# acbull/pyHGT

Hardware: AMD Instinct MI355X
Metric: HGTConv forward edges/sec (higher is better)
Workload: dtype f32 (typed linears and relation transforms as 3-term fp16 hi/lo MFMA with power-of-two row scales, fp32 accumulate)

## Files before the change

include/hgt_hip.h:

```cpp
#ifndef HGT_HIP_H_
#define HGT_HIP_H_

#include <stddef.h>
#include <stdint.h>

#ifdef __cplusplus
extern "C" {
#endif

#define HGT_ABI_VERSION 8

#define HGT_OK 0
#define HGT_ERR_INVALID_ARG (-1)
#define HGT_ERR_UNSUPPORTED (-2)
#define HGT_ERR_WORKSPACE (-3)
#define HGT_ERR_TOO_LARGE (-4)
#define HGT_ERR_LAUNCH (-5)

#define HGT_RTE_LEN 240

const char* hgt_strerror(int code);
int hgt_abi_version(void);
#define HGT_FEATURE_DETERMINISTIC_TRAINING 2
int hgt_build_features(void);
// ... 76 lines not shown
int hgt_linear_update_f16x3(const float* agg, int64_t ld_agg, const int32_t* rows, const int32_t* group_off,
                            int32_t n_groups, int64_t n_rows, int32_t k, int32_t n_out, const void* w_split,
                            const float* bias, int64_t b_group_stride, const float* x_skip, int64_t ld_skip,
                            const float* skip, const float* ln_w, const float* ln_b, int32_t use_norm, float* out,
                            void* stream);
int hgt_zero_rows(const int32_t* rows, const int32_t* range, int32_t d, float* out, void* stream);

int hgt_relation_pack(const float* relation_att, const float* relation_msg, const float* relation_pri,
                      int32_t n_relations, int32_t n_heads, int32_t n_heads_layout, int32_t d_k, int32_t dk_pad,
                      float* att_t, float* msg_p, void* stream);

int hgt_edge_logits(const void* plan, int64_t n_nodes, int64_t n_edges, int32_t n_types, int32_t n_relations,
                    int32_t n_heads, int32_t dk_pad, const float* Q, const float* K, const float* rte_k,
                    const float* att_t, float* logits, void* stream);
int hgt_edge_logits_mfma(const void* plan, int64_t n_nodes, int64_t n_edges, int32_t n_types, int32_t n_relations,
                         int32_t n_heads, int32_t dk_pad, const float* Q, const float* K, const float* rte_k,
                         const float* att_t, const void* att_frag, int32_t frag_f16, float* logits, void* stream);
int hgt_relation_kside_bytes(int32_t n_relations, int32_t n_heads, int32_t dk_pad, uint64_t* out_host);
int hgt_relation_kside_pack(const float* att_t, int32_t n_relations, int32_t n_heads, int32_t dk_pad, void* att_kside, void* stream);
int hgt_edge_logits_kside(const void* plan, int64_t n_nodes, int64_t n_edges, int32_t n_types, int32_t n_relations,
                          int32_t n_heads, int32_t dk_pad, const float* Q, const float* K, const float* rte_k,
                          const float* att_t, const void* att_kside, int32_t frag_f16, float* logits, void* stream);
int hgt_kside_image_map(int32_t n_blocks, int32_t* image_map, int32_t* b_col, int32_t* c_out);
int hgt_edge_logits_range(const void* plan, int64_t n_nodes, int64_t n_edges, int32_t n_types, int32_t n_relations,
                          int32_t n_heads, int32_t dk_pad, const float* Q, const float* K, const float* rte_k,
                          const float* att_t, const void* att_frag, int32_t frag_f16, float* logits, int32_t item_begin,
                          int32_t item_end, void* stream);
int hgt_edge_softmax(const void* plan, int64_t n_nodes, int64_t n_edges, int32_t n_types, int32_t n_relations,
                     int32_t n_heads, float* logits_att, void* stream);
int hgt_edge_aggregate(const void* plan, int64_t n_nodes, int64_t n_edges, int32_t n_types, int32_t n_relations,
                       int32_t n_heads, int32_t dk_pad, const float* logits, const float* V, const float* rte_v,
                       const float* msg_p, const void* msg_frag, float* agg, int64_t n_q_rows, int32_t apply_gelu,
                       void* hub_ws, void* stream);
int hgt_edge_aggregate_items_bytes(int64_t n_edges, int32_t n_heads, int32_t dk_pad, uint64_t* out_host);
int hgt_edge_aggregate_items(const void* plan, int64_t n_nodes, int64_t n_edges, int32_t n_types, int32_t n_relations,
                             int32_t n_heads, int32_t dk_pad, const float* logits, const float* V, const float* rte_v,
                             const void* msg_frag, int32_t frag_f16, float* agg, int64_t n_q_rows, int32_t apply_gelu,
                             void* scratch, uint64_t scratch_bytes, void* stream);
int hgt_edge_aggregate_items_update(const void* plan, int64_t n_nodes, int64_t n_edges, int32_t n_types, int32_t n_relations,
                                    int32_t n_heads, int32_t dk_pad, const float* logits, const float* V, const float* rte_v,
                                    const void* msg_frag, int32_t frag_f16, int64_t n_q_rows, void* scratch, uint64_t scratch_bytes,
                                    const int32_t* rows, const int32_t* group_off, int32_t n_groups, const void* w_a_split,
                                    const float* b_a, const float* x_skip, int64_t ld_skip, const float* skip, const float* ln_w,
                                    const float* ln_b, int32_t use_norm, int32_t n_out, float* out, void* stream);
int hgt_edge_logits_slice(const void* plan, int64_t n_nodes, int64_t n_edges, int32_t n_types, int32_t n_relations,
                          int32_t n_heads, int32_t dk_pad, const float* Q, const float* K, const float* rte_k,
// ... 169 lines not shown
    int32_t stage;
    const int32_t* proj_rows;
    const int32_t* proj_off;
    int64_t proj_n;
    void* prepared;
    uint64_t prepared_bytes;
    int32_t prepared_valid;
    int32_t plan_no_hubs;
    int32_t flags;
    int32_t slice_index;
    int32_t slice_count;
    int64_t q_begin, q_end;
    int32_t item_begin, item_end;
    const void* proj_c24;
    int64_t proj_c24_row0;
} hgt_conv_args;

#define HGT_FLAG_NO_FUSED_UPDATE 1
#define HGT_FLAG_VALU_AGGREGATE  2
#define HGT_FLAG_MFMA_LOGITS     4
#define HGT_FLAG_VALU_LOGITS     8
#define HGT_FLAG_KSIDE_LOGITS 65536
#define HGT_FLAG_NO_KSIDE_LOGITS 131072
#define HGT_FLAG_ITEM_AGGREGATE 16
#define HGT_FLAG_NO_ITEM_AGGREGATE 32
#define HGT_FLAG_FUSED_ANY_SIZE 64
#define HGT_FLAG_XS_GEMM_ALWAYS 1024
#define HGT_FLAG_XS_GEMM_NEVER 2048
#define HGT_FLAG_NO_TILE_GEMM 4096
#define HGT_FLAG_NO_MERGE_UPDATE 8192
#define HGT_FLAG_NO_COOP_EDGE 16384
#define HGT_FLAG_COOP_EDGE_ALWAYS 32768
#define HGT_FLAG_DETERMINISTIC_HUBS 128

#define HGT_N_PHASE_EVENTS 7

int hgt_conv_workspace_bytes(int64_t n_nodes, int64_t n_edges, int32_t in_dim, int32_t out_dim,
                             int32_t n_types, int32_t n_relations, int32_t n_heads, int32_t use_rte,
                             uint64_t* out_host);
int hgt_conv_workspace_bytes_ex(int64_t n_nodes, int64_t n_edges, int32_t in_dim, int32_t out_dim,
                                int32_t n_types, int32_t n_relations, int32_t n_heads, int32_t use_rte, int32_t options,
                                uint64_t* out_host);
int hgt_conv_prepared_bytes(int32_t in_dim, int32_t out_dim, int32_t n_types, int32_t n_relations, int32_t n_heads,
                            int32_t use_rte, uint64_t* out_host);
int hgt_conv_forward(const hgt_conv_args* args_host, void* stream);

// ... 181 lines not shown
```

pyhgt_amd/_lib.py:

```python
import ctypes as C
import os

_HERE = os.path.dirname(os.path.abspath(__file__))
LIB_PATH = os.environ.get("HGT_LIB_PATH", os.path.join(_HERE, "lib", "libhgt_hip.so"))

HGT_RTE_LEN = 240
HGT_N_PHASE_EVENTS = 7
HGT_FLAG_NO_FUSED_UPDATE = 1
HGT_FLAG_VALU_AGGREGATE = 2
HGT_FLAG_MFMA_LOGITS = 4
HGT_FLAG_VALU_LOGITS = 8
HGT_FLAG_ITEM_AGGREGATE = 16
HGT_FLAG_NO_ITEM_AGGREGATE = 32
HGT_FLAG_FUSED_ANY_SIZE = 64
HGT_FLAG_DETERMINISTIC_HUBS = 128
HGT_FLAG_XS_GEMM_ALWAYS = 1024
HGT_FLAG_XS_GEMM_NEVER = 2048
HGT_FLAG_NO_TILE_GEMM = 4096
HGT_FLAG_NO_MERGE_UPDATE = 8192
HGT_FLAG_NO_COOP_EDGE = 16384
HGT_FLAG_COOP_EDGE_ALWAYS = 32768
HGT_FLAG_KSIDE_LOGITS = 65536
HGT_FLAG_NO_KSIDE_LOGITS = 131072
HGT_LINEAR_FORCE_XS = 0x100
HGT_LINEAR_NO_XS = 0x200
HGT_LINEAR_NO_TILE = 0x400
HGT_LINEAR_TANH = 0x1000
HGT_FEATURE_DETERMINISTIC_TRAINING = 2
HGT_STACK_MAX_PIECES = 256
HGT_SAMPLER_MAX_TYPES = 16
HGT_SAMPLER_MAX_TRIPLES = 48
HGT_SAMPLER_MAX_NUMBER = 1024
HGT_SAMPLER_HUB_DEG = 512
HGT_SAMPLER_TIME_NONE = -2 ** 31
HGT_SAMPLER_MAX_BATCH = 64


class HgtLayout(C.Structure):
    _fields_ = [("d_k", C.c_int32), ("dk_pad", C.c_int32), ("d_pad", C.c_int32), ("vec", C.c_int32), ("heads", C.c_int32)]


class HgtPlanSizes(C.Structure):
    _fields_ = [("plan_bytes", C.c_uint64), ("tmp_bytes", C.c_uint64), ("max_items", C.c_int64), ("n_bins", C.c_int64)]


class HgtPlanRows(C.Structure):
# ... 73 lines not shown
    "hgt_plan_from_sorted": (C.c_int, [_vp, _vp, _vp, _vp, _vp, _i64, _i64, _i64, _i32, _i32, _vp, _u64, _vp, _u64, _vp]),
    "hgt_typed_linear": (C.c_int, [_vp, _i64, _vp, _vp, _i32, _i64, _i32, _i32, _vp, _i64, _vp, _i64, _vp, _vp, _vp,
                                   _i32, _i32, _i32, _i32, _vp]),
    "hgt_split_weights_bytes": (C.c_int, [_i32, _i32, _i32, C.POINTER(_u64)]),
    "hgt_split_weights": (C.c_int, [_vp, _i64, _i32, _i32, _i32, _vp, _vp]),
    "hgt_typed_linear_bf16x3": (C.c_int, [_vp, _i64, _vp, _vp, _i32, _i64, _i32, _i32, _vp, _vp, _i64, _vp, _vp, _vp,
                                          _i32, _i32, _i32, _vp]),
    "hgt_linear_update_bf16x3": (C.c_int, [_vp, _i64, _vp, _vp, _i32, _i64, _i32, _i32, _vp, _vp, _i64, _vp, _i64, _vp, _vp, _vp,
                                           _i32, _vp, _vp]),
    "hgt_split_weights_f16": (C.c_int, [_vp, _i64, _i32, _i32, _i32, _vp, _vp]),
    "hgt_typed_linear_xs_schedule": (C.c_int, [_vp, _i32, _i64, _i32, _i32, _vp, _i64, C.POINTER(_i64)]),
    "hgt_typed_linear_f16x3": (C.c_int, [_vp, _i64, _vp, _vp, _i32, _i64, _i32, _i32, _vp, _vp, _i64, _vp, _vp, _vp,
                                         _i32, _i32, _i32, _vp]),
    "hgt_linear_update_f16x3": (C.c_int, [_vp, _i64, _vp, _vp, _i32, _i64, _i32, _i32, _vp, _vp, _i64, _vp, _i64, _vp, _vp, _vp,
                                          _i32, _vp, _vp]),
    "hgt_zero_rows": (C.c_int, [_vp, _vp, _i32, _vp, _vp]),
    "hgt_relation_pack": (C.c_int, [_vp, _vp, _vp, _i32, _i32, _i32, _i32, _i32, _vp, _vp, _vp]),
    "hgt_edge_logits": (C.c_int, [_vp, _i64, _i64, _i32, _i32, _i32, _i32, _vp, _vp, _vp, _vp, _vp, _vp]),
    "hgt_edge_logits_mfma": (C.c_int, [_vp, _i64, _i64, _i32, _i32, _i32, _i32, _vp, _vp, _vp, _vp, _vp, _i32, _vp, _vp]),
    "hgt_relation_kside_bytes": (C.c_int, [_i32, _i32, _i32, C.POINTER(_u64)]),
    "hgt_relation_kside_pack": (C.c_int, [_vp, _i32, _i32, _i32, _vp, _vp]),
    "hgt_edge_logits_kside": (C.c_int, [_vp, _i64, _i64, _i32, _i32, _i32, _i32, _vp, _vp, _vp, _vp, _vp, _i32, _vp, _vp]),
    "hgt_kside_image_map": (C.c_int, [_i32, _vp, _vp, _vp]),
    "hgt_edge_logits_range": (C.c_int, [_vp, _i64, _i64, _i32, _i32, _i32, _i32, _vp, _vp, _vp, _vp, _vp, _i32, _vp, _i32, _i32, _vp]),
    "hgt_edge_aggregate_update_range": (C.c_int, [_vp, _i64, _i64, _i32, _i32, _i32, _i32, _vp, _vp, _vp, _vp, _vp, _vp, _i64, _vp, _vp, _vp,
                                                  _vp, _vp, _vp, _i64, _vp, _vp, _vp, _i32, _i32, _vp, _vp, _i64, _i64, _i32, _i32]),
    "hgt_hub_workspace_bytes_ex": (C.c_int, [_i64, _i32, _i32, _i32, _i32, C.POINTER(_u64)]),
    "hgt_edge_aggregate_ex": (C.c_int, [_vp, _i64, _i64, _i32, _i32, _i32, _i32, _vp, _vp, _vp, _vp, _vp, _i32, _vp, _i64, _i32, _vp, _i32, _vp]),
    "hgt_edge_logits_slice": (C.c_int, [_vp, _i64, _i64, _i32, _i32, _i32, _i32, _vp, _vp, _vp, _vp, _vp, _i32, _i32, _vp]),
    "hgt_edge_aggregate_slice": (C.c_int, [_vp, _i64, _i64, _i32, _i32, _i32, _i32, _vp, _vp, _vp, _vp, _vp, _vp, _i64, _i32, _vp,
                                           _i32, _i32, _vp, _i32, _i32, _vp]),
    "hgt_edge_aggregate_slice_ex": (C.c_int, [_vp, _i64, _i64, _i32, _i32, _i32, _i32, _vp, _vp, _vp, _vp, _vp, _vp, _i64, _i32, _vp,
                                              _i32, _i32, _vp, _i32, _i32, _i32, _vp]),
    "hgt_edge_softmax": (C.c_int, [_vp, _i64, _i64, _i32, _i32, _i32, _vp, _vp]),
    "hgt_edge_aggregate": (C.c_int, [_vp, _i64, _i64, _i32, _i32, _i32, _i32, _vp, _vp, _vp, _vp, _vp, _vp, _i64, _i32, _vp, _vp]),
    "hgt_edge_aggregate_f16x3": (C.c_int, [_vp, _i64, _i64, _i32, _i32, _i32, _i32, _vp, _vp, _vp, _vp, _vp, _vp, _i64, _i32, _vp, _vp]),
    "hgt_relation_frag_pack_f16": (C.c_int, [_vp, _i32, _i32, _i32, _vp, _vp]),
    "hgt_edge_aggregate_items_bytes": (C.c_int, [_i64, _i32, _i32, C.POINTER(_u64)]),
    "hgt_edge_spmm_items": (C.c_int, [_vp, _i64, _i64, _i32, _i32, _i32, _i32, _vp, _vp, _vp, _vp, _vp, _i64, _i64, _vp, _u64, _vp]),
    "hgt_edge_aggregate_items_update": (C.c_int, [_vp, _i64, _i64, _i32, _i32, _i32, _i32, _vp, _vp, _vp, _vp, _i32, _i64, _vp, _u64, _vp, _vp, _i32,
                                                  _vp, _vp, _vp, _i64, _vp, _vp, _vp, _i32, _i32, _vp, _vp]),
    "hgt_edge_aggregate_items": (C.c_int, [_vp, _i64, _i64, _i32, _i32, _i32, _i32, _vp, _vp, _vp, _vp, _i32, _vp, _i64, _i32, _vp, _u64, _vp]),
    "hgt_plan_header_to_host": (C.c_int, [_vp, _vp, _vp]),
    "hgt_relation_frag_bytes": (C.c_int, [_i32, _i32, _i32, C.POINTER(_u64)]),
    "hgt_relation_frag_pack": (C.c_int, [_vp, _i32, _i32, _i32, _vp, _vp]),
    "hgt_hub_workspace_bytes": (C.c_int, [_i64, _i32, _i32, C.POINTER(_u64)]),
# ... 127 lines not shown
```

pyhgt_amd/csrc/hgt_api.hip:

```cpp
#include "hgt_common.h"

#ifndef HGT_FUSED_MIN_NODES
#define HGT_FUSED_MIN_NODES 16384
#endif
#ifndef HGT_ITEM_AGG_MAX_NODES
#define HGT_ITEM_AGG_MAX_NODES 65536
#endif
#ifndef HGT_ITEM_AGG_DEFAULT_NODES
#define HGT_ITEM_AGG_DEFAULT_NODES 65536
#endif

int hgt_edge_logits_kside_items(const void* plan, int64_t N, int64_t E, int32_t T, int32_t R, int32_t H, int32_t dk_pad, const float* Q,
                                const float* K, const float* rte_k, const void* att_kside, float* logits, int item_lo, int item_hi, void* stream);

namespace {

struct ConvWorkspace {
    uint64_t off_q, off_k, off_v, off_logits, off_agg, off_trans, off_att_t, off_msg_p, off_msg_f, off_att_f, off_att_k, off_hub;
    uint64_t off_rte_lin, off_rte_k, off_rte_v, off_rte_rows, off_rte_off, off_ws_qkv, off_ws_a, off_ws_rte, off_off2, off_pending, off_state, off_zitems, zitems_bytes, total;
    void drop_item_scratch() { zitems_bytes = 0; total = off_zitems; }
};

static ConvWorkspace conv_workspace(int64_t N, int64_t NQ, int64_t E, int in_dim, int out_dim, int T, int R, int , int use_rte,
                                    const hgt_layout& lay, bool item_scratch = true, bool det_hubs = false) {
    const int H = lay.heads;
    ConvWorkspace w;
    uint64_t o = 0;
    auto take = [&](uint64_t bytes) { uint64_t r = o; o = hgt_align_up(o + bytes, 256); return r; };
    const uint64_t dp = (uint64_t)lay.d_pad;
    w.off_q = take((uint64_t)NQ * dp * 4);
    w.off_k = take((uint64_t)N * dp * 4);
    w.off_v = take((uint64_t)N * dp * 4);
    w.off_logits = take((uint64_t)E * H * 4);
    w.off_agg = take((uint64_t)NQ * dp * 4);
    w.off_trans = take((uint64_t)NQ * out_dim * 4);
    w.off_att_t = take((uint64_t)R * H * lay.dk_pad * lay.dk_pad * 4);
// ... 273 lines not shown
                          a->b_qkv, 3 * dp, Q, K, V, dp, 0, ws_qkv, 0, !fresh);
        int rc = linear(a->x, din, pr.rows_q, pr.off_q, T, NQ, din, dp, a->w_qkv, wstride, a->b_qkv, 3 * dp, Q, nullptr, nullptr, dp, 0, ws_a);
        if (rc != HGT_OK) return rc;
        rc = linear(a->x, din, pr.rows_all, pr.off_all, T, N, din, 2 * dp, a->w_qkv + (int64_t)dp * din, wstride, a->b_qkv + dp, 3 * dp,
                    K, V, nullptr, dp, 0, wb + w.off_ws_qkv);
        if (rc != HGT_OK || !(a->prepared && fresh && split)) return rc;
        return split_weights(a->w_qkv, wstride, T, din, 3 * dp, ws_qkv, stream);
    }

    int temporal_tables() const {
        if (!a->use_rte || !fresh) return HGT_OK;
        float* rte_lin = (float*)(wb + w.off_rte_lin);
        int32_t* rrows = (int32_t*)(wb + w.off_rte_rows);
        int32_t* roff = (int32_t*)(wb + w.off_rte_off);
        k_rte_row_lists<<<(T * HGT_RTE_LEN + 255) / 256, 256, 0, stream>>>(T, rrows, roff);
        int rc = linear(a->rte_emb, din, rrows, roff, 1, HGT_RTE_LEN, din, din, a->rte_w, 0, a->rte_b, 0, rte_lin, nullptr, nullptr, din, 1,
                        wb + w.off_ws_rte);
        if (rc != HGT_OK) return rc;
        return linear(rte_lin, din, rrows, roff, T, (int64_t)T * HGT_RTE_LEN, din, 2 * dp, a->w_qkv + (int64_t)dp * din, (int64_t)3 * dp * din,
                      nullptr, 0, rte_k, rte_v, nullptr, dp, 1, ws_a);
    }

    int edge_logits() const {
        if (r.logits == LOGITS_KSIDE) {
            const int rc = hgt_edge_logits_kside(a->plan, N, E, T, R, H, dkp, Q, K, rte_k, att_t, att_k_buf, fmode, logits, stream);
            if (rc != HGT_ERR_UNSUPPORTED) return rc;
            if (r.mfma_logits) return hgt_edge_logits_mfma(a->plan, N, E, T, R, H, dkp, Q, K, rte_k, att_t, att_f_buf, fmode, logits, stream);
        }
        switch (r.logits) {
            case LOGITS_RANGE:
                if (r.kside_range) {
                    const int rc = hgt_edge_logits_kside_items(a->plan, N, E, T, R, H, dkp, Q, K, rte_k, att_k_buf, logits, a->item_begin, a->item_end, stream);
                    if (rc != HGT_ERR_UNSUPPORTED) return rc;
                }
                return hgt_edge_logits_range(a->plan, N, E, T, R, H, dkp, Q, K, rte_k, att_t, r.mfma_logits ? att_f_buf : nullptr, fmode, logits,
                                             a->item_begin, a->item_end, stream);
            case LOGITS_SLICE: return hgt_edge_logits_slice(a->plan, N, E, T, R, H, dkp, Q, K, rte_k, att_t, logits, sl_lo, sl_hi, stream);
            case LOGITS_MFMA: return hgt_edge_logits_mfma(a->plan, N, E, T, R, H, dkp, Q, K, rte_k, att_t, att_f_buf, fmode, logits, stream);
            default: return hgt_edge_logits(a->plan, N, E, T, R, H, dkp, Q, K, rte_k, att_t, logits, stream);
        }
    }

    int aggregate_update(int64_t q0, int64_t q1, int hub_det) const {
        return hgt_edge_aggregate_update_sel(a->plan, N, E, T, R, H, dkp, logits, V, rte_v, msg_p, msg_f, agg, NQ, hub_ws,
                                             (int32_t*)(wb + w.off_pending), a->node_type, ws_upd, a->b_a, a->x, din, a->skip, a->ln_w,
                                             a->ln_b, a->use_norm, dout, a->out, stream, q0, q1, f16 ? 1 : 0, hub_det);
    }

    int aggregate(AggForm form) const {
        void* zitems = wb + w.off_zitems;
        switch (form) {
            case AGG_FUSED:
                if (det_hubs && hub_ws && !msg_f)
                    return HGT_ERR_UNSUPPORTED;
                return aggregate_update(0, (det_hubs && hub_ws) ? NQ : -1, (det_hubs && hub_ws) ? 1 : 0);
// ... 164 lines not shown
```

pyhgt_amd/csrc/hgt_edge_logits_kside.hip:

```cpp
#include "hgt_edge_common.h"
#include "hgt_split_common.h"
#include "hgt_kside_map.h"

namespace {

typedef unsigned hgt_u32x2 __attribute__((ext_vector_type(2)));

__device__ __forceinline__ void half_pair(unsigned x, unsigned& lo, unsigned& up) {
#if __has_builtin(__builtin_amdgcn_permlane32_swap)
    const hgt_u32x2 r = __builtin_amdgcn_permlane32_swap(x, x, false, false);
    lo = r[0];
    up = r[1];
#else
    const unsigned o = (unsigned)__shfl_xor((int)x, 32);
    const bool upper = (threadIdx.x & 32) != 0;
    lo = upper ? o : x;
    up = upper ? x : o;
#endif
}
__device__ __forceinline__ unsigned half_max_bits(unsigned x) {
    unsigned a, b;
    half_pair(x, a, b);
    return max(a, b);
}
// ... 30 lines not shown
    const float* blk = attT + (int64_t)rh * HGT_KSIDE_DK * HGT_KSIDE_DK;
    unsigned m = 0u;
#pragma unroll
    for (int q = 0; q < 4; ++q) m = max(m, __builtin_bit_cast(unsigned, fabsf(blk[t + 256 * q])));
    m = wave_max_bits(m);
    if ((t & 63) == 0) s_m[t >> 6] = m;
    __syncthreads();
    m = max(max(s_m[0], s_m[1]), max(s_m[2], s_m[3]));
    const int e = kside_exp(m);
    const float scale = kside_scale(e);
#pragma unroll
    for (int q = 0; q < 4; ++q) {
        const int p = t + 256 * q;
        const int j = p & 7, lane = (p >> 3) & 63, s = p >> 9;
        const float v = blk[hgt_kside_image_out(lane) * HGT_KSIDE_DK + hgt_kside_image_k(s, lane, j)];
        unsigned short hi, lo;
        split1_t<true>(v, scale, hi, lo);
        img[hgt_kside_image_index(rh, s, 0, lane, j)] = hi;
        img[hgt_kside_image_index(rh, s, 1, lane, j)] = lo;
    }
    if (t == 0) reinterpret_cast<int*>(img + (int64_t)n_rh * HGT_KSIDE_BLOCK_ELEMS)[rh] = e - 141;
}

struct KsideRows {
    float4 k[4], q[4];
};

typedef unsigned hgt_u32x4 __attribute__((ext_vector_type(4)));
typedef __amdgpu_buffer_rsrc_t kside_rsrc;

__device__ __forceinline__ kside_rsrc kside_table(const float* p, unsigned bytes) {
    return __builtin_amdgcn_make_buffer_rsrc(const_cast<float*>(p), 0, (int)bytes, 0x00020000);
}
__device__ __forceinline__ float4 kside_load16(kside_rsrc t, unsigned off) {
    const hgt_u32x4 v = __builtin_amdgcn_raw_buffer_load_b128(t, (int)off, 0, 0);
    return __builtin_bit_cast(float4, v);
}

template <int H>
__device__ __forceinline__ void kside_issue(kside_rsrc K, kside_rsrc Q, unsigned koff, unsigned qoff, int h, KsideRows& b) {
#pragma unroll
    for (int i = 0; i < 4; ++i) b.k[i] = kside_load16(K, koff + h * 128 + 16 * i);
#pragma unroll
    for (int i = 0; i < 4; ++i) b.q[i] = kside_load16(Q, qoff + h * 128 + 16 * i);
}

__device__ __forceinline__ float kside_head(const KsideRows& b, const hgt_f16x8 (&ah)[2], const hgt_f16x8 (&al)[2], int ea) {
    const int ek = kside_exp(half_max_bits(abs_bits16(b.k)));
    const float ks = kside_scale(ek);
    hgt_f16x8 kh[2], kl[2];
#pragma unroll
    for (int s = 0; s < 2; ++s) {
        static_assert(hgt_kside_k_col(1, 0, 0) == 8 && hgt_kside_k_col(0, 1, 0) == 16, "k-step s takes floats 8 s .. 8 s + 7 of the lane's piece");
        uint4 hi, lo;
        split2_f16(b.k[2 * s].x * ks, b.k[2 * s].y * ks, hi.x, lo.x);
        split2_f16(b.k[2 * s].z * ks, b.k[2 * s].w * ks, hi.y, lo.y);
        split2_f16(b.k[2 * s + 1].x * ks, b.k[2 * s + 1].y * ks, hi.z, lo.z);
        split2_f16(b.k[2 * s + 1].z * ks, b.k[2 * s + 1].w * ks, hi.w, lo.w);
        kh[s] = __builtin_bit_cast(hgt_f16x8, hi);
        kl[s] = __builtin_bit_cast(hgt_f16x8, lo);
    }
    f32x16 acc = {0.f, 0.f, 0.f, 0.f, 0.f, 0.f, 0.f, 0.f, 0.f, 0.f, 0.f, 0.f, 0.f, 0.f, 0.f, 0.f};
    acc = __builtin_amdgcn_mfma_f32_32x32x16_f16(al[0], kh[0], acc, 0, 0, 0);
    acc = __builtin_amdgcn_mfma_f32_32x32x16_f16(al[1], kh[1], acc, 0, 0, 0);
    acc = __builtin_amdgcn_mfma_f32_32x32x16_f16(ah[0], kl[0], acc, 0, 0, 0);
    acc = __builtin_amdgcn_mfma_f32_32x32x16_f16(ah[1], kl[1], acc, 0, 0, 0);
    acc = __builtin_amdgcn_mfma_f32_32x32x16_f16(ah[0], kh[0], acc, 0, 0, 0);
    acc = __builtin_amdgcn_mfma_f32_32x32x16_f16(ah[1], kh[1], acc, 0, 0, 0);
    int eq = (int)(half_max_bits(abs_bits16(b.q)) >> 23);
    eq = eq < 1 ? 1 : (eq > 253 ? 253 : eq);
    const float qs = __builtin_bit_cast(float, (unsigned)(254 - eq) << 23);
    static_assert(hgt_kside_c_out(1, 5) == 21, "register reg of the accumulator is output 16 half + reg: the lane's own Q piece");
    const hgt_f32x2 qs2 = {qs, qs};
    hgt_f32x2 d = {0.0f, 0.0f};
#pragma unroll
    for (int i = 0; i < 4; ++i) {
        const hgt_f32x2 q0 = {b.q[i].x, b.q[i].y}, q1 = {b.q[i].z, b.q[i].w};
        const hgt_f32x2 a0 = {acc[4 * i], acc[4 * i + 1]}, a1 = {acc[4 * i + 2], acc[4 * i + 3]};
        d = __builtin_elementwise_fma(q0 * qs2, a0, d);
        d = __builtin_elementwise_fma(q1 * qs2, a1, d);
    }
    const float d0 = d[0], d1 = d[1];
    return ldexpf(half_sum(d0 + d1), (eq - 127) + (ek - 141) + ea);
}

template <int H>
__global__ __launch_bounds__(256, 2) void k_edge_logits_kside(
    const HgtItem* __restrict__ items, const HgtPlanHeader* __restrict__ hdr, const int32_t* __restrict__ esrc,
    const int32_t* __restrict__ edst, const float* __restrict__ Qp, const float* __restrict__ Kp, unsigned table_bytes,
    const unsigned short* __restrict__ img, float* __restrict__ logits, int R, int item_lo, int item_hi, int items_cap) {
    static_assert(H == 2 || H == 4 || H == 8, "one head group of 32-column heads");
    constexpr int HW = H < 4 ? H : 4, WPI = H / HW;
    constexpr unsigned ROWB = H * 128;
    const int lane = threadIdx.x & 63;
    const int wib = __builtin_amdgcn_readfirstlane(threadIdx.x >> 6);
    const int item = item_lo + hgt_item_block() * (4 / WPI) + wib / WPI;
    const int h0 = (wib % WPI) * HW;
    const HgtItem it = items[min(item, items_cap - 1)];
    if (item >= (item_hi >= 0 ? item_hi : hdr->n_items)) return;
    const int beg = __builtin_amdgcn_readfirstlane(it.beg), end = __builtin_amdgcn_readfirstlane(it.end);
    const int rel = __builtin_amdgcn_readfirstlane(it.rel);
    if (beg >= end) return;
    if (rel >= R) {
        if (h0 == 0)
            for (int64_t i = (int64_t)beg * H + lane; i < (int64_t)end * H; i += 64) logits[i] = 0.0f;
        return;
    }
    const int el = lane & 31, half = lane >> 5;
    const kside_rsrc K = kside_table(Kp, table_bytes), Q = kside_table(Qp, table_bytes);

    hgt_f16x8 ah[HW][2], al[HW][2];
    {
        const uint4* ip = reinterpret_cast<const uint4*>(img) + ((int64_t)rel * H + h0) * 256 + lane;
#pragma unroll
        for (int h = 0; h < HW; ++h)
#pragma unroll
            for (int s = 0; s < 2; ++s) {
                ah[h][s] = __builtin_bit_cast(hgt_f16x8, ip[((h * 2 + s) * 2 + 0) * 64]);
                al[h][s] = __builtin_bit_cast(hgt_f16x8, ip[((h * 2 + s) * 2 + 1) * 64]);
            }
    }
    const int* eap = reinterpret_cast<const int*>(img + (int64_t)R * H * HGT_KSIDE_BLOCK_ELEMS) + rel * H + h0;
    int ea[HW];
#pragma unroll
    for (int h = 0; h < HW; ++h) ea[h] = eap[h];

    const unsigned lo = (unsigned)half * 64u + (unsigned)h0 * 128u;
    int li = min(beg + el, end - 1);
    unsigned koff = (unsigned)esrc[li] * ROWB + lo, qoff = (unsigned)edst[li] * ROWB + lo;
    li = min(beg + 32 + el, end - 1);
    unsigned koff_n = (unsigned)esrc[li] * ROWB + lo, qoff_n = (unsigned)edst[li] * ROWB + lo;
    KsideRows buf[HW];
#pragma unroll
    for (int h = 0; h < HW - 1; ++h) kside_issue<H>(K, Q, koff, qoff, h, buf[h]);
    li = min(beg + 64 + el, end - 1);
    int s2 = esrc[li], d2 = edst[li];
    for (int base = beg; base < end; base += 32) {
        float lg[HW];
#pragma unroll
        for (int h = 0; h < HW; ++h) {
            if (h == 0) kside_issue<H>(K, Q, koff, qoff, HW - 1, buf[HW - 1]);
            else kside_issue<H>(K, Q, koff_n, qoff_n, h - 1, buf[h - 1]);
            __builtin_amdgcn_sched_barrier(0);
            lg[h] = kside_head(buf[h], ah[h], al[h], ea[h]);
            __builtin_amdgcn_sched_barrier(0);
        }
        if (half == 0 && base + el < end) {
            float* o = logits + (int64_t)(base + el) * H + h0;
            if constexpr (HW == 2) *reinterpret_cast<float2*>(o) = make_float2(lg[0], lg[1]);
            else *reinterpret_cast<float4*>(o) = make_float4(lg[0], lg[1], lg[2], lg[3]);
        }
        koff = koff_n;
        qoff = qoff_n;
        koff_n = (unsigned)s2 * ROWB + lo;
        qoff_n = (unsigned)d2 * ROWB + lo;
        li = min(base + 96 + el, end - 1);
        s2 = esrc[li];
        d2 = edst[li];
    }
}

template <int H>
static void launch_kside(const HgtPlanView& pv, const float* Q, const float* K, unsigned table_bytes, const unsigned short* img, float* logits, int R,
                         int item_lo, int item_hi, hipStream_t stream) {
    constexpr int IPW = H == 8 ? 2 : 4;
    const int64_t n_launch = item_hi >= 0 ? (int64_t)(item_hi - item_lo) : pv.L.max_items;
    const unsigned blocks = hgt_item_grid((n_launch + IPW - 1) / IPW);
    k_edge_logits_kside<H><<<blocks, 256, 0, stream>>>(pv.items, pv.hdr, pv.esrc, pv.edst, Q, K, table_bytes, img, logits, R, item_lo, item_hi, (int)pv.L.max_items);
}

static bool kside_layout(int32_t H, int32_t dk_pad) { return dk_pad == HGT_KSIDE_DK && (H == 2 || H == 4 || H == 8); }

}

extern "C" int hgt_relation_kside_bytes(int32_t R, int32_t H, int32_t dk_pad, uint64_t* out) {
    if (!out || R <= 0 || H <= 0 || dk_pad <= 0) return HGT_ERR_INVALID_ARG;
    *out = kside_layout(H, dk_pad) ? (uint64_t)R * H * HGT_KSIDE_BLOCK_ELEMS * 2 + hgt_align_up((uint64_t)R * H * 4, 256) : 0;
    return HGT_OK;
}

extern "C" int hgt_relation_kside_pack(const float* att_t, int32_t R, int32_t H, int32_t dk_pad, void* att_kside, void* stream) {
    if (!att_t || !att_kside || R <= 0 || H <= 0 || dk_pad <= 0) return HGT_ERR_INVALID_ARG;
    if (!kside_layout(H, dk_pad)) return HGT_ERR_UNSUPPORTED;
    k_relation_kside_pack<<<(unsigned)(R * H), 256, 0, (hipStream_t)stream>>>(att_t, R * H, (unsigned short*)att_kside);
    HGT_CHECK_LAUNCH();
    return HGT_OK;
}

__attribute__((visibility("hidden"))) int hgt_edge_logits_kside_items(const void* plan, int64_t N, int64_t E, int32_t T, int32_t R, int32_t H,
                                                                      int32_t dk_pad, const float* Q, const float* K, const float* rte_k,
                                                                      const void* att_kside, float* logits, int item_lo, int item_hi, void* stream) {
    if (!plan || !Q || !K || !att_kside || (E > 0 && !logits) || N < 0 || E < 0 || R <= 0 || H <= 0 || 64 % H != 0 || dk_pad <= 0)
        return HGT_ERR_INVALID_ARG;
    if (dk_pad % (64 / H) != 0) return HGT_ERR_INVALID_ARG;
    if (!kside_layout(H, dk_pad) || rte_k || (uint64_t)N * (uint64_t)H * (uint64_t)dk_pad * 4u >= (1ull << 32)) return HGT_ERR_UNSUPPORTED;
    if (E == 0) return HGT_OK;
    const HgtPlanView pv = hgt_plan_view(plan, N, E, T, R);
    const unsigned short* img = (const unsigned short*)att_kside;
    const unsigned table_bytes = (unsigned)((uint64_t)N * H * dk_pad * 4u);
    if (H == 2) launch_kside<2>(pv, Q, K, table_bytes, img, logits, R, item_lo, item_hi, (hipStream_t)stream);
    else if (H == 4) launch_kside<4>(pv, Q, K, table_bytes, img, logits, R, item_lo, item_hi, (hipStream_t)stream);
    else launch_kside<8>(pv, Q, K, table_bytes, img, logits, R, item_lo, item_hi, (hipStream_t)stream);
    HGT_CHECK_LAUNCH();
    return HGT_OK;
}

extern "C" int hgt_edge_logits_kside(const void* plan, int64_t N, int64_t E, int32_t T, int32_t R, int32_t H, int32_t dk_pad,
                                     const float* Q, const float* K, const float* rte_k, const float* att_t, const void* att_kside,
                                     int32_t frag_f16, float* logits, void* stream) {
    (void)att_t;
    (void)frag_f16;
    return hgt_edge_logits_kside_items(plan, N, E, T, R, H, dk_pad, Q, K, rte_k, att_kside, logits, 0, -1, stream);
}

extern "C" int hgt_kside_image_map(int32_t n_blocks, int32_t* image_map, int32_t* b_col, int32_t* c_out) {
    if (n_blocks < 0) return HGT_ERR_INVALID_ARG;
    if (image_map)
        for (int64_t rh = 0; rh < n_blocks; ++rh)
            for (int s = 0; s < 2; ++s)
                for (int term = 0; term < 2; ++term)
                    for (int lane = 0; lane < 64; ++lane)
                        for (int j = 0; j < 8; ++j) {
                            int32_t* o = image_map + 4 * hgt_kside_image_index(rh, s, term, lane, j);
                            o[0] = (int32_t)rh, o[1] = term, o[2] = hgt_kside_image_out(lane), o[3] = hgt_kside_image_k(s, lane, j);
                        }
    for (int lane = 0; lane < 64; ++lane) {
        if (b_col)
            for (int s = 0; s < 2; ++s)
                for (int j = 0; j < 8; ++j) b_col[(s * 64 + lane) * 8 + j] = hgt_kside_k_col(s, lane >> 5, j);
        if (c_out)
            for (int reg = 0; reg < 16; ++reg) c_out[lane * 16 + reg] = hgt_kside_c_out(lane >> 5, reg);
    }
    return HGT_OK;
}
```

pyhgt_amd/csrc/hgt_kside_map.h:

```cpp
#pragma once
#include <stdint.h>

#if defined(__HIPCC__) || defined(__CUDACC__)
#define HGT_KSIDE_HD __host__ __device__
#else
#define HGT_KSIDE_HD
#endif

constexpr int HGT_KSIDE_DK = 32;
constexpr int HGT_KSIDE_BLOCK_ELEMS = 2 * 2 * 64 * 8;

HGT_KSIDE_HD constexpr int hgt_kside_row_out(int m) { return 16 * ((m >> 2) & 1) + (m & 3) + 4 * (m >> 3); }
HGT_KSIDE_HD constexpr int hgt_kside_k_col(int s, int half, int j) { return 16 * half + 8 * s + j; }
HGT_KSIDE_HD constexpr int hgt_kside_c_out(int half, int reg) { return hgt_kside_row_out((reg & 3) + 8 * (reg >> 2) + 4 * half); }

HGT_KSIDE_HD constexpr int64_t hgt_kside_image_index(int64_t rh, int s, int term, int lane, int j) {
    return (((rh * 2 + s) * 2 + term) * 64 + lane) * 8 + j;
}
HGT_KSIDE_HD constexpr int hgt_kside_image_out(int lane) { return hgt_kside_row_out(lane & 31); }
HGT_KSIDE_HD constexpr int hgt_kside_image_k(int s, int lane, int j) { return hgt_kside_k_col(s, lane >> 5, j); }

static_assert(hgt_kside_c_out(0, 0) == 0 && hgt_kside_c_out(0, 15) == 15 && hgt_kside_c_out(1, 0) == 16 && hgt_kside_c_out(1, 15) == 31,
              "a lane receives 16 consecutive outputs");
```

Measured before the change: 1.462 billion.

## Gather K/Q rows into an LDS ring via buffer-load-to-LDS DMA in kside logits

The kside edge-logits kernel gets a new default path that gathers K and Q rows with `buffer_load_dwordx4 ... lds` DMAs into a two-slot ring in shared memory per wave. Edge ids are redistributed across lanes with ds_bpermute, and a swizzled chunk layout is used so each lane then reads its fragments from LDS. Loads for head h+2, or the next edge batch, are issued while head h is computed, replacing the register-buffered per-lane buffer loads. The old register path is kept behind a flag. The new path adds inline asm that manipulates m0 and hand-placed vmcnt waits, plus LDS usage that may lower occupancy, and it derives the path selection from a bit of frag_f16.

```diff
diff --git a/include/hgt_hip.h b/include/hgt_hip.h
--- a/include/hgt_hip.h
+++ b/include/hgt_hip.h
@@ -122,6 +122,7 @@
                           int32_t n_heads, int32_t dk_pad, const float* Q, const float* K, const float* rte_k,
                           const float* att_t, const void* att_kside, int32_t frag_f16, float* logits, void* stream);
 int hgt_kside_image_map(int32_t n_blocks, int32_t* image_map, int32_t* b_col, int32_t* c_out);
+int hgt_kside_gather_map(int32_t* dma_map, int32_t* read_map);
 int hgt_edge_logits_range(const void* plan, int64_t n_nodes, int64_t n_edges, int32_t n_types, int32_t n_relations,
                           int32_t n_heads, int32_t dk_pad, const float* Q, const float* K, const float* rte_k,
                           const float* att_t, const void* att_frag, int32_t frag_f16, float* logits, int32_t item_begin,
@@ -337,6 +338,7 @@
 #define HGT_FLAG_VALU_LOGITS     8
 #define HGT_FLAG_KSIDE_LOGITS 65536
 #define HGT_FLAG_NO_KSIDE_LOGITS 131072
+#define HGT_FLAG_KSIDE_LANE_GATHER 262144
 #define HGT_FLAG_ITEM_AGGREGATE 16
 #define HGT_FLAG_NO_ITEM_AGGREGATE 32
 #define HGT_FLAG_FUSED_ANY_SIZE 64
diff --git a/pyhgt_amd/_lib.py b/pyhgt_amd/_lib.py
--- a/pyhgt_amd/_lib.py
+++ b/pyhgt_amd/_lib.py
@@ -22,6 +22,7 @@
 HGT_FLAG_COOP_EDGE_ALWAYS = 32768
 HGT_FLAG_KSIDE_LOGITS = 65536
 HGT_FLAG_NO_KSIDE_LOGITS = 131072
+HGT_FLAG_KSIDE_LANE_GATHER = 262144
 HGT_LINEAR_FORCE_XS = 0x100
 HGT_LINEAR_NO_XS = 0x200
 HGT_LINEAR_NO_TILE = 0x400
@@ -141,6 +142,7 @@
     "hgt_relation_kside_pack": (C.c_int, [_vp, _i32, _i32, _i32, _vp, _vp]),
     "hgt_edge_logits_kside": (C.c_int, [_vp, _i64, _i64, _i32, _i32, _i32, _i32, _vp, _vp, _vp, _vp, _vp, _i32, _vp, _vp]),
     "hgt_kside_image_map": (C.c_int, [_i32, _vp, _vp, _vp]),
+    "hgt_kside_gather_map": (C.c_int, [_vp, _vp]),
     "hgt_edge_logits_range": (C.c_int, [_vp, _i64, _i64, _i32, _i32, _i32, _i32, _vp, _vp, _vp, _vp, _vp, _i32, _vp, _i32, _i32, _vp]),
     "hgt_edge_aggregate_update_range": (C.c_int, [_vp, _i64, _i64, _i32, _i32, _i32, _i32, _vp, _vp, _vp, _vp, _vp, _vp, _i64, _vp, _vp, _vp,
                                                   _vp, _vp, _vp, _i64, _vp, _vp, _vp, _i32, _i32, _vp, _vp, _i64, _i64, _i32, _i32]),
diff --git a/pyhgt_amd/csrc/hgt_api.hip b/pyhgt_amd/csrc/hgt_api.hip
--- a/pyhgt_amd/csrc/hgt_api.hip
+++ b/pyhgt_amd/csrc/hgt_api.hip
@@ -11,7 +11,8 @@
 #endif
 
 int hgt_edge_logits_kside_items(const void* plan, int64_t N, int64_t E, int32_t T, int32_t R, int32_t H, int32_t dk_pad, const float* Q,
-                                const float* K, const float* rte_k, const void* att_kside, float* logits, int item_lo, int item_hi, void* stream);
+                                const float* K, const float* rte_k, const void* att_kside, float* logits, int item_lo, int item_hi, int lane_gather,
+                                void* stream);
 
 namespace {
 
@@ -331,15 +332,16 @@
     }
 
     int edge_logits() const {
+        const int kside_lane = (a->flags & HGT_FLAG_KSIDE_LANE_GATHER) ? 8 : 0;
         if (r.logits == LOGITS_KSIDE) {
-            const int rc = hgt_edge_logits_kside(a->plan, N, E, T, R, H, dkp, Q, K, rte_k, att_t, att_k_buf, fmode, logits, stream);
+            const int rc = hgt_edge_logits_kside(a->plan, N, E, T, R, H, dkp, Q, K, rte_k, att_t, att_k_buf, fmode | kside_lane, logits, stream);
             if (rc != HGT_ERR_UNSUPPORTED) return rc;
             if (r.mfma_logits) return hgt_edge_logits_mfma(a->plan, N, E, T, R, H, dkp, Q, K, rte_k, att_t, att_f_buf, fmode, logits, stream);
         }
         switch (r.logits) {
             case LOGITS_RANGE:
                 if (r.kside_range) {
-                    const int rc = hgt_edge_logits_kside_items(a->plan, N, E, T, R, H, dkp, Q, K, rte_k, att_k_buf, logits, a->item_begin, a->item_end, stream);
+                    const int rc = hgt_edge_logits_kside_items(a->plan, N, E, T, R, H, dkp, Q, K, rte_k, att_k_buf, logits, a->item_begin, a->item_end, kside_lane, stream);
                     if (rc != HGT_ERR_UNSUPPORTED) return rc;
                 }
                 return hgt_edge_logits_range(a->plan, N, E, T, R, H, dkp, Q, K, rte_k, att_t, r.mfma_logits ? att_f_buf : nullptr, fmode, logits,
diff --git a/pyhgt_amd/csrc/hgt_edge_logits_kside.hip b/pyhgt_amd/csrc/hgt_edge_logits_kside.hip
--- a/pyhgt_amd/csrc/hgt_edge_logits_kside.hip
+++ b/pyhgt_amd/csrc/hgt_edge_logits_kside.hip
@@ -76,11 +76,12 @@
     if (t == 0) reinterpret_cast<int*>(img + (int64_t)n_rh * HGT_KSIDE_BLOCK_ELEMS)[rh] = e - 141;
 }
 
+typedef unsigned hgt_u32x4 __attribute__((ext_vector_type(4)));
+
 struct KsideRows {
     float4 k[4], q[4];
 };
 
-typedef unsigned hgt_u32x4 __attribute__((ext_vector_type(4)));
 typedef __amdgpu_buffer_rsrc_t kside_rsrc;
 
 __device__ __forceinline__ kside_rsrc kside_table(const float* p, unsigned bytes) {
@@ -97,6 +98,47 @@
     for (int i = 0; i < 4; ++i) b.k[i] = kside_load16(K, koff + h * 128 + 16 * i);
 #pragma unroll
     for (int i = 0; i < 4; ++i) b.q[i] = kside_load16(Q, qoff + h * 128 + 16 * i);
+}
+
+constexpr unsigned KSIDE_PIECE = 1024;
+constexpr unsigned KSIDE_SIDE = 4 * KSIDE_PIECE;
+constexpr unsigned KSIDE_SLOT = 2 * KSIDE_SIDE;
+constexpr unsigned KSIDE_RING = 2;
+constexpr unsigned KSIDE_WAVE_LDS = KSIDE_RING * KSIDE_SLOT;
+
+__device__ __forceinline__ hgt_u32x4 kside_table_words(const float* p, unsigned bytes) {
+    const uint64_t a = (uint64_t)(uintptr_t)p;
+    const hgt_u32x4 r = {(unsigned)a, (unsigned)(a >> 32) & 0xffffu, bytes, 0x00020000u};
+    return r;
+}
+__device__ __forceinline__ void kside_dma4(hgt_u32x4 table, const unsigned (&voff)[4], unsigned soff, unsigned lds_dst) {
+    unsigned keep;
+    asm volatile(
+        "s_nop 1\n\ts_mov_b32 %0, m0\n\t"
+        "s_mov_b32 m0, %6\n\ts_nop 0\n\tbuffer_load_dwordx4 %1, %5, %7 offen lds\n\t"
+        "s_add_u32 m0, %6, 0x400\n\ts_nop 0\n\tbuffer_load_dwordx4 %2, %5, %7 offen lds\n\t"
+        "s_add_u32 m0, %6, 0x800\n\ts_nop 0\n\tbuffer_load_dwordx4 %3, %5, %7 offen lds\n\t"
+        "s_add_u32 m0, %6, 0xc00\n\ts_nop 0\n\tbuffer_load_dwordx4 %4, %5, %7 offen lds\n\t"
+        "s_mov_b32 m0, %0"
+        : "=&s"(keep)
+        : "v"(voff[0]), "v"(voff[1]), "v"(voff[2]), "v"(voff[3]), "s"(table), "s"(lds_dst), "s"(soff)
+        : "memory", "scc");
+}
+static_assert(KSIDE_PIECE == 0x400, "the piece stride written into kside_dma4");
+constexpr int KSIDE_STEP_DMAS = 8;
+__device__ __forceinline__ void kside_wait_vm() { asm volatile("s_waitcnt vmcnt(8)" ::: "memory"); }
+__device__ __forceinline__ void kside_wait_vm_ids(int& s, int& d) { asm volatile("s_waitcnt vmcnt(8)" : "+v"(s), "+v"(d) : : "memory"); }
+__device__ __forceinline__ void kside_ids_request(const int32_t* ps, const int32_t* pd, int& s, int& d) {
+    asm volatile("global_load_dword %0, %2, off\n\tglobal_load_dword %1, %3, off" : "=&v"(s), "=&v"(d) : "v"(ps), "v"(pd) : "memory");
+}
+__device__ __forceinline__ void kside_wait_lds() { asm volatile("s_waitcnt lgkmcnt(0)" ::: "memory"); }
+
+__device__ __forceinline__ void kside_piece_offsets(int s, int d, const int (&bp)[4], const unsigned (&cp)[4], unsigned rowb, unsigned (&off)[8]) {
+#pragma unroll
+    for (int p = 0; p < 4; ++p) {
+        off[p] = (unsigned)__builtin_amdgcn_ds_bpermute(bp[p], s) * rowb + cp[p];
+        off[4 + p] = (unsigned)__builtin_amdgcn_ds_bpermute(bp[p], d) * rowb + cp[p];
+    }
 }
 
 __device__ __forceinline__ float kside_head(const KsideRows& b, const hgt_f16x8 (&ah)[2], const hgt_f16x8 (&al)[2], int ea) {
@@ -138,7 +180,7 @@
     return ldexpf(half_sum(d0 + d1), (eq - 127) + (ek - 141) + ea);
 }
 
-template <int H>
+template <int H, bool LANE>
 __global__ __launch_bounds__(256, 2) void k_edge_logits_kside(
     const HgtItem* __restrict__ items, const HgtPlanHeader* __restrict__ hdr, const int32_t* __restrict__ esrc,
     const int32_t* __restrict__ edst, const float* __restrict__ Qp, const float* __restrict__ Kp, unsigned table_bytes,
@@ -161,7 +203,6 @@
         return;
     }
     const int el = lane & 31, half = lane >> 5;
-    const kside_rsrc K = kside_table(Kp, table_bytes), Q = kside_table(Qp, table_bytes);
 
     hgt_f16x8 ah[HW][2], al[HW][2];
     {
@@ -179,48 +220,124 @@
 #pragma unroll
     for (int h = 0; h < HW; ++h) ea[h] = eap[h];
 
-    const unsigned lo = (unsigned)half * 64u + (unsigned)h0 * 128u;
-    int li = min(beg + el, end - 1);
-    unsigned koff = (unsigned)esrc[li] * ROWB + lo, qoff = (unsigned)edst[li] * ROWB + lo;
-    li = min(beg + 32 + el, end - 1);
-    unsigned koff_n = (unsigned)esrc[li] * ROWB + lo, qoff_n = (unsigned)edst[li] * ROWB + lo;
-    KsideRows buf[HW];
-#pragma unroll
-    for (int h = 0; h < HW - 1; ++h) kside_issue<H>(K, Q, koff, qoff, h, buf[h]);
-    li = min(beg + 64 + el, end - 1);
-    int s2 = esrc[li], d2 = edst[li];
-    for (int base = beg; base < end; base += 32) {
-        float lg[HW];
-#pragma unroll
-        for (int h = 0; h < HW; ++h) {
-            if (h == 0) kside_issue<H>(K, Q, koff, qoff, HW - 1, buf[HW - 1]);
-            else kside_issue<H>(K, Q, koff_n, qoff_n, h - 1, buf[h - 1]);
-            __builtin_amdgcn_sched_barrier(0);
-            lg[h] = kside_head(buf[h], ah[h], al[h], ea[h]);
-            __builtin_amdgcn_sched_barrier(0);
+    if constexpr (LANE) {
+        const kside_rsrc K = kside_table(Kp, table_bytes), Q = kside_table(Qp, table_bytes);
+        const unsigned lo = (unsigned)half * 64u + (unsigned)h0 * 128u;
+        int li = min(beg + el, end - 1);
+        unsigned koff = (unsigned)esrc[li] * ROWB + lo, qoff = (unsigned)edst[li] * ROWB + lo;
+        li = min(beg + 32 + el, end - 1);
+        unsigned koff_n = (unsigned)esrc[li] * ROWB + lo, qoff_n = (unsigned)edst[li] * ROWB + lo;
+        KsideRows buf[HW];
+#pragma unroll
+        for (int h = 0; h < HW - 1; ++h) kside_issue<H>(K, Q, koff, qoff, h, buf[h]);
+        li = min(beg + 64 + el, end - 1);
+        int s2 = esrc[li], d2 = edst[li];
+        for (int base = beg; base < end; base += 32) {
+            float lg[HW];
+#pragma unroll
+            for (int h = 0; h < HW; ++h) {
+                if (h == 0) kside_issue<H>(K, Q, koff, qoff, HW - 1, buf[HW - 1]);
+                else kside_issue<H>(K, Q, koff_n, qoff_n, h - 1, buf[h - 1]);
+                __builtin_amdgcn_sched_barrier(0);
+                lg[h] = kside_head(buf[h], ah[h], al[h], ea[h]);
+                __builtin_amdgcn_sched_barrier(0);
+            }
+            if (half == 0 && base + el < end) {
+                float* o = logits + (int64_t)(base + el) * H + h0;
+                if constexpr (HW == 2) *reinterpret_cast<float2*>(o) = make_float2(lg[0], lg[1]);
+                else *reinterpret_cast<float4*>(o) = make_float4(lg[0], lg[1], lg[2], lg[3]);
+            }
+            koff = koff_n;
+            qoff = qoff_n;
+            koff_n = (unsigned)s2 * ROWB + lo;
+            qoff_n = (unsigned)d2 * ROWB + lo;
+            li = min(base + 96 + el, end - 1);
+            s2 = esrc[li];
+            d2 = edst[li];
         }
-        if (half == 0 && base + el < end) {
-            float* o = logits + (int64_t)(base + el) * H + h0;
-            if constexpr (HW == 2) *reinterpret_cast<float2*>(o) = make_float2(lg[0], lg[1]);
-            else *reinterpret_cast<float4*>(o) = make_float4(lg[0], lg[1], lg[2], lg[3]);
+    } else {
+        static_assert(HW % 2 == 0 && KSIDE_RING == 2 && KSIDE_STEP_DMAS == 8, "slot of a step = its head & 1; eight DMAs per step");
+        __shared__ __attribute__((aligned(1024))) unsigned char ring[4 * KSIDE_WAVE_LDS];
+        const unsigned lds_wave = __builtin_amdgcn_readfirstlane((unsigned)(uintptr_t)(__attribute__((address_space(3))) unsigned char*)ring) +
+                                  (unsigned)wib * KSIDE_WAVE_LDS;
+        const unsigned char* rd = ring + (unsigned)wib * KSIDE_WAVE_LDS;
+        const hgt_u32x4 K = kside_table_words(Kp, table_bytes), Q = kside_table_words(Qp, table_bytes);
+        unsigned cp[4], ra[4];
+        int bp[4];
+#pragma unroll
+        for (int p = 0; p < 4; ++p) {
+            cp[p] = (unsigned)h0 * 128u + 16u * (unsigned)hgt_kside_dma_chunk(p, lane);
+            bp[p] = 4 * hgt_kside_dma_edge(p, lane);
+            ra[p] = (unsigned)hgt_kside_read_offset(lane, p);
         }
-        koff = koff_n;
-        qoff = qoff_n;
-        koff_n = (unsigned)s2 * ROWB + lo;
-        qoff_n = (unsigned)d2 * ROWB + lo;
-        li = min(base + 96 + el, end - 1);
-        s2 = esrc[li];
-        d2 = edst[li];
+        unsigned off_c[8], off_n[8];
+        int li = min(beg + el, end - 1);
+        kside_piece_offsets(esrc[li], edst[li], bp, cp, ROWB, off_c);
+        li = min(beg + 32 + el, end - 1);
+        kside_piece_offsets(esrc[li], edst[li], bp, cp, ROWB, off_n);
+#pragma unroll
+        for (int h = 0; h < HW; ++h)
+#pragma unroll
+            for (int s = 0; s < 2; ++s) asm volatile("" : "+v"(ah[h][s]), "+v"(al[h][s]));
+#pragma unroll
+        for (int h = 0; h < HW; ++h) asm volatile("" : "+v"(ea[h]));
+#pragma unroll
+        for (int i = 0; i < 8; ++i) asm volatile("" : "+v"(off_c[i]), "+v"(off_n[i]));
+#pragma unroll
+        for (int h = 0; h < 2; ++h) {
+            kside_dma4(K, reinterpret_cast<const unsigned(&)[4]>(off_c[0]), h * 128u, lds_wave + h * KSIDE_SLOT);
+            kside_dma4(Q, reinterpret_cast<const unsigned(&)[4]>(off_c[4]), h * 128u, lds_wave + h * KSIDE_SLOT + KSIDE_SIDE);
+        }
+        int s2 = 0, d2 = 0;
+        for (int base = beg; base < end; base += 32) {
+            float lg[HW];
+#pragma unroll
+            for (int h = 0; h < HW; ++h) {
+                const unsigned slot = (h & 1) * KSIDE_SLOT;
+                if (h == 1) kside_wait_vm_ids(s2, d2);
+                else kside_wait_vm();
+                KsideRows b;
+#pragma unroll
+                for (int i = 0; i < 4; ++i) {
+                    b.k[i] = *reinterpret_cast<const float4*>(rd + slot + ra[i]);
+                    b.q[i] = *reinterpret_cast<const float4*>(rd + slot + KSIDE_SIDE + ra[i]);
+                }
+                kside_wait_lds();
+                if (h == 0) {
+                    li = min(base + 64 + el, end - 1);
+                    kside_ids_request(esrc + li, edst + li, s2, d2);
+                }
+                const bool same = h + 2 < HW;
+                const unsigned hn = (same ? h + 2 : h + 2 - HW) * 128u;
+                kside_dma4(K, reinterpret_cast<const unsigned(&)[4]>(same ? off_c[0] : off_n[0]), hn, lds_wave + slot);
+                kside_dma4(Q, reinterpret_cast<const unsigned(&)[4]>(same ? off_c[4] : off_n[4]), hn, lds_wave + slot + KSIDE_SIDE);
+                __builtin_amdgcn_sched_barrier(0);
+                lg[h] = kside_head(b, ah[h], al[h], ea[h]);
+                __builtin_amdgcn_sched_barrier(0);
+            }
+            if (half == 0 && base + el < end) {
+                float* o = logits + (int64_t)(base + el) * H + h0;
+                if constexpr (HW == 2) *reinterpret_cast<float2*>(o) = make_float2(lg[0], lg[1]);
+                else *reinterpret_cast<float4*>(o) = make_float4(lg[0], lg[1], lg[2], lg[3]);
+            }
+#pragma unroll
+            for (int i = 0; i < 8; ++i) off_c[i] = off_n[i];
+            kside_piece_offsets(s2, d2, bp, cp, ROWB, off_n);
+        }
+        asm volatile("s_waitcnt vmcnt(0)" ::: "memory");
     }
 }
 
 template <int H>
 static void launch_kside(const HgtPlanView& pv, const float* Q, const float* K, unsigned table_bytes, const unsigned short* img, float* logits, int R,
-                         int item_lo, int item_hi, hipStream_t stream) {
+                         int item_lo, int item_hi, bool lane_gather, hipStream_t stream) {
     constexpr int IPW = H == 8 ? 2 : 4;
     const int64_t n_launch = item_hi >= 0 ? (int64_t)(item_hi - item_lo) : pv.L.max_items;
     const unsigned blocks = hgt_item_grid((n_launch + IPW - 1) / IPW);
-    k_edge_logits_kside<H><<<blocks, 256, 0, stream>>>(pv.items, pv.hdr, pv.esrc, pv.edst, Q, K, table_bytes, img, logits, R, item_lo, item_hi, (int)pv.L.max_items);
+    if (lane_gather)
+        k_edge_logits_kside<H, true><<<blocks, 256, 0, stream>>>(pv.items, pv.hdr, pv.esrc, pv.edst, Q, K, table_bytes, img, logits, R, item_lo, item_hi, (int)pv.L.max_items);
+    else
+        k_edge_logits_kside<H, false><<<blocks, 256, 0, stream>>>(pv.items, pv.hdr, pv.esrc, pv.edst, Q, K, table_bytes, img, logits, R, item_lo, item_hi, (int)pv.L.max_items);
 }
 
 static bool kside_layout(int32_t H, int32_t dk_pad) { return dk_pad == HGT_KSIDE_DK && (H == 2 || H == 4 || H == 8); }
@@ -243,7 +360,8 @@
 
 __attribute__((visibility("hidden"))) int hgt_edge_logits_kside_items(const void* plan, int64_t N, int64_t E, int32_t T, int32_t R, int32_t H,
                                                                       int32_t dk_pad, const float* Q, const float* K, const float* rte_k,
-                                                                      const void* att_kside, float* logits, int item_lo, int item_hi, void* stream) {
+                                                                      const void* att_kside, float* logits, int item_lo, int item_hi, int lane_gather,
+                                                                      void* stream) {
     if (!plan || !Q || !K || !att_kside || (E > 0 && !logits) || N < 0 || E < 0 || R <= 0 || H <= 0 || 64 % H != 0 || dk_pad <= 0)
         return HGT_ERR_INVALID_ARG;
     if (dk_pad % (64 / H) != 0) return HGT_ERR_INVALID_ARG;
@@ -252,9 +370,9 @@
     const HgtPlanView pv = hgt_plan_view(plan, N, E, T, R);
     const unsigned short* img = (const unsigned short*)att_kside;
     const unsigned table_bytes = (unsigned)((uint64_t)N * H * dk_pad * 4u);
-    if (H == 2) launch_kside<2>(pv, Q, K, table_bytes, img, logits, R, item_lo, item_hi, (hipStream_t)stream);
-    else if (H == 4) launch_kside<4>(pv, Q, K, table_bytes, img, logits, R, item_lo, item_hi, (hipStream_t)stream);
-    else launch_kside<8>(pv, Q, K, table_bytes, img, logits, R, item_lo, item_hi, (hipStream_t)stream);
+    if (H == 2) launch_kside<2>(pv, Q, K, table_bytes, img, logits, R, item_lo, item_hi, lane_gather != 0, (hipStream_t)stream);
+    else if (H == 4) launch_kside<4>(pv, Q, K, table_bytes, img, logits, R, item_lo, item_hi, lane_gather != 0, (hipStream_t)stream);
+    else launch_kside<8>(pv, Q, K, table_bytes, img, logits, R, item_lo, item_hi, lane_gather != 0, (hipStream_t)stream);
     HGT_CHECK_LAUNCH();
     return HGT_OK;
 }
@@ -263,8 +381,7 @@
                                      const float* Q, const float* K, const float* rte_k, const float* att_t, const void* att_kside,
                                      int32_t frag_f16, float* logits, void* stream) {
     (void)att_t;
-    (void)frag_f16;
-    return hgt_edge_logits_kside_items(plan, N, E, T, R, H, dk_pad, Q, K, rte_k, att_kside, logits, 0, -1, stream);
+    return hgt_edge_logits_kside_items(plan, N, E, T, R, H, dk_pad, Q, K, rte_k, att_kside, logits, 0, -1, frag_f16 & 8, stream);
 }
 
 extern "C" int hgt_kside_image_map(int32_t n_blocks, int32_t* image_map, int32_t* b_col, int32_t* c_out) {
@@ -287,3 +404,18 @@
     }
     return HGT_OK;
 }
+
+extern "C" int hgt_kside_gather_map(int32_t* dma_map, int32_t* read_map) {
+    for (int lane = 0; lane < 64; ++lane)
+        for (int p = 0; p < 4; ++p) {
+            if (dma_map) {
+                int32_t* o = dma_map + 2 * (p * 64 + lane);
+                o[0] = hgt_kside_dma_edge(p, lane), o[1] = hgt_kside_dma_chunk(p, lane);
+            }
+            if (read_map) {
+                int32_t* o = read_map + 3 * (p * 64 + lane);
+                o[0] = hgt_kside_read_offset(lane, p), o[1] = lane & 31, o[2] = hgt_kside_read_chunk(lane, p);
+            }
+        }
+    return HGT_OK;
+}
diff --git a/pyhgt_amd/csrc/hgt_kside_map.h b/pyhgt_amd/csrc/hgt_kside_map.h
--- a/pyhgt_amd/csrc/hgt_kside_map.h
+++ b/pyhgt_amd/csrc/hgt_kside_map.h
@@ -22,3 +22,14 @@
 
 static_assert(hgt_kside_c_out(0, 0) == 0 && hgt_kside_c_out(0, 15) == 15 && hgt_kside_c_out(1, 0) == 16 && hgt_kside_c_out(1, 15) == 31,
               "a lane receives 16 consecutive outputs");
+
+HGT_KSIDE_HD constexpr int hgt_kside_gather_swizzle(int p, int r) { return 2 * (p & 3) + ((r >> 1) & 1); }
+HGT_KSIDE_HD constexpr int hgt_kside_gather_slot(int p, int r, int c) { return 8 * r + (c ^ hgt_kside_gather_swizzle(p, r)); }
+HGT_KSIDE_HD constexpr int hgt_kside_dma_edge(int p, int s) { return 8 * p + (s >> 3); }
+HGT_KSIDE_HD constexpr int hgt_kside_dma_chunk(int p, int s) { return (s & 7) ^ hgt_kside_gather_swizzle(p, s >> 3); }
+HGT_KSIDE_HD constexpr int hgt_kside_read_chunk(int lane, int i) { return 4 * (lane >> 5) + i; }
+HGT_KSIDE_HD constexpr int hgt_kside_read_offset(int lane, int i) {
+    return 1024 * ((lane & 31) >> 3) + 16 * hgt_kside_gather_slot((lane & 31) >> 3, lane & 7, hgt_kside_read_chunk(lane, i));
+}
+static_assert(hgt_kside_gather_slot(3, 7, hgt_kside_dma_chunk(3, 61)) == 61 && hgt_kside_dma_edge(3, 61) == 31,
+              "a DMA lane fetches the chunk that belongs in its own slot");
```

Result: faster. 1.501 billion (median of 6 runs) (+2.7%).
